# osqp/OSQP.jl

Hardware: AMD Instinct MI355X
Metric: ADMM iterations/sec (higher is better)
Workload: dtype f64; 1 GPU; rand-1e6; n=1000000, m=1000000, nnz_A=1000000000, nnz_P_full=1000749500, nnz_P_triu=500874750, backend=pcg, check_termination=25, adaptive_rho_interval=50, instances=1

## Files before the change

### osqp.jl_amd/csrc/abi.hip

```cpp
#include "engine.hpp"
#include "symbolic.hpp"

#include <cstring>
#include <thread>
#include <atomic>
#include <cmath>

using namespace oq;

namespace {

struct Impl {
  Engine eng;
  OSQPData data;
  OSQPSettings settings;
  OSQPSolution solution;
  OSQPInfo info;
};

Engine *E(OSQPWorkspace *w) { return &((Impl *)w->impl)->eng; }

struct DeviceGuard {
  int prev = -1;
  explicit DeviceGuard(int want) {
// ... 378 lines not shown
              const int k = R.rowid[r];
              same = k >= 0 && k < S.N && !seen[k];
              if (!same) break;
              seen[k] = 1;
              const int64_t len = S.Rp[k + 1] - S.Rp[k];
              same = c + (size_t)len <= R.cols[b].size();
              if (!same) break;
              std::vector<int> got(R.cols[b].begin() + c, R.cols[b].begin() + c + len);
              std::sort(got.begin(), got.end());
              same = std::equal(got.begin(), got.end(), S.Rj.begin() + S.Rp[k]);
              c += (size_t)len;
            }
          }
        }
        Supernodes T2;
        build_supernodes(S2, (int)smax, T2, false, true);
        same = same && T2.count == T.count && T2.ptr == T.ptr && T2.piv == T.piv && T2.up == T.up && T2.lvl_ptr == T.lvl_ptr && T2.woff == T.woff;
        for (int q = 0; q < S.N && same; q++) same = T2.Fp[q + 1] - T2.Fp[q] >= T.Fp[q + 1] - T.Fp[q] && T2.Gp[q + 1] - T2.Gp[q] >= T.Gp[q + 1] - T.Gp[q];
      }
      symbolic_complete(S2);
      same = same && !S2.lean && S2.Lp == S.Lp && S2.Li == S.Li && S2.Rp == S.Rp && S2.Rj == S.Rj && S2.Rmap == S.Rmap && S2.PtoL == S.PtoL &&
             S2.AtoL == S.AtoL;
      out[14] = same ? 1.0 : 0.0;
    }
    out[5] = (double)T.Fp[S.N]; out[6] = (double)T.wdoubles; out[7] = largest; out[8] = ok ? 1.0 : 0.0; out[9] = (double)inside;
    int lD, cD, kD;
    choose_dense_top(S, 512, getenv("OSQP_AMD_DENSE_MAX") ? atoi(getenv("OSQP_AMD_DENSE_MAX")) : 12288, 1024, 32, lD, cD, kD);
    out[10] = level_solve_cost_us(S, 512, lD, kD); out[11] = supernode_solve_cost_us(T, 256);
    out[12] = supernodes_pay(S, T, 512, lD, kD, 256) ? 1.0 : 0.0;
    if (getenv("OSQP_AMD_PROBE_VERBOSE"))
      for (int L = 0; L < T.nlev; L++) {
        int64_t rows = 0, pre = 0, post = 0, back = 0;
        int smax_l = 0;
        for (int J = T.lvl_ptr[L]; J < T.lvl_ptr[L + 1]; J++) {
          smax_l = std::max(smax_l, T.ptr[J + 1] - T.ptr[J]);
          for (int q = T.ptr[J]; q < T.ptr[J + 1]; q++) { rows++; pre += T.Fsplit[q] - T.Fp[q]; post += T.Fp[q + 1] - T.Fsplit[q]; back += T.Gp[q + 1] - T.Gp[q]; }
        }
        {
          int64_t cnt[3] = {0, 0, 0}, rw[3] = {0, 0, 0}, ef[3] = {0, 0, 0}, eb[3] = {0, 0, 0}, mxb[3] = {0, 0, 0};
          for (int J = T.lvl_ptr[L]; J < T.lvl_ptr[L + 1]; J++) {
            const int64_t sz = T.ptr[J + 1] - T.ptr[J];
            const int c = sz == 1 ? 0 : (sz <= Supernodes::kSmall ? 1 : 2);
            cnt[c]++; rw[c] += sz;
            for (int q = T.ptr[J]; q < T.ptr[J + 1]; q++) { ef[c] += T.Fp[q + 1] - T.Fp[q]; eb[c] += T.Gp[q + 1] - T.Gp[q]; mxb[c] = std::max<int64_t>(mxb[c], T.Gp[q + 1] - T.Gp[q]); }
          }
          for (int c = 0; c < 3; c++)
// ... 300 lines not shown
```

### osqp.jl_amd/csrc/direct.hip

```cpp
#include <climits>
#include <cstring>
#include <cmath>

#include "engine.hpp"
#include "symbolic.hpp"
#include "mfront.hpp"
#include "mfront_big.hpp"

namespace oq {

namespace {

constexpr int kChainRows = 512;
constexpr int kChainThreads = 1024;

}
}

#include "direct_factor_kernels.hpp"
#include "direct_dense_kernels.hpp"
#include "direct_level_kernels.hpp"
#include "direct_sn_kernels.hpp"
#include "direct_sndense_kernels.hpp"

// ... 19 lines not shown
  double *Sinv = nullptr;
  int ldD = 0;
  std::vector<char> long_rows;
  size_t w_half = 0;
  std::vector<Step> fwd, bwd;
  long long factorizations = 0;
  bool sn = false;
  Supernodes T;
  DevBuf<int> sn_ptr, sn_piv, perm_s, pinv_s, sn_Fj, sn_Gi, sn_up, sn_waits, sn_pending, sn_ready;
  int *sn_fault = nullptr, *sn_fault_host = nullptr;
  ~LdlFactor() { if (sn_fault_host) (void)hipHostFree(sn_fault_host); }
  bool faulted() const {
    if (!sn_fault_host) return false;
    if (inject_fault) { inject_fault = false; *sn_fault_host = 1; }
    return *(volatile int *)sn_fault_host != 0;
  }
  mutable bool inject_fault = getenv("OSQP_AMD_SNODE_FAULT_TEST") && atoi(getenv("OSQP_AMD_SNODE_FAULT_TEST")) == 1;
  bool sn_tree = false;
  int sn_tree_threads = 1024;
  int sn_tree_grid = 0;
  DevBuf<int> sn_ticket;
  int sn_tree_L0 = 1;
  DevBuf<int64_t> sn_woff, sn_wmap, sn_Fp, sn_Fpos, sn_Gp, sn_Gpos, sn_Fsplit;
  DevBuf<double> sn_Wc, sn_Wr, sn_Fx, sn_Gx, sn_Dinv;
  std::vector<int> sn_lanes_f, sn_lanes_b;
  bool mf = false;
  DevBuf<int> mf_snof, mf_slot, mf_bsz, mf_chp, mf_chl, mf_list, mf_err;
  DevBuf<int64_t> mf_uoff, mf_reloff;
  DevBuf<uint16_t> mf_rel, mf_loc;
  DevBuf<double> mf_U;
  struct MfLaunch { int cls, off, count, fcap; int tile_off = 0, tile_count = 0, chunk_off = 0, chunk_count = 0; };
  std::vector<MfLaunch> mf_launches;
  DevBuf<int64_t> mf_poff;
  DevBuf<double> mf_panel;
  DevBuf<int64_t> mf_ct0;
  DevBuf<int> mf_tiles, mf_chunks, mf_wide, mf_nwide;
  std::vector<int> mfh_chunks;
  std::vector<int64_t> mfh_poff;
  std::vector<char> mf_is_big;
  std::vector<int> mfh_tiles;
  int mf_big_count = 0, mf_big_fmax = 0;
  int mf_fmax = 0;
  bool mf_ok = false;
  int snd_L0 = -1, snd_J0 = -1, snd_q0 = 0, snd_K = 0;
  int snd_nb = 0, snd_nv = 0, snd_ntiles = 0;
  bool snd_vec_mode = false;
// ... 243 lines not shown
      HIP_CHECK(hipHostGetDevicePointer((void **)&sn_fault, sn_fault_host, 0));
    }
    up64(sn_woff, T.woff);
    if (lean) lean_device_lists(q_upper);
    else {
      if (!mf_ok) up64(sn_wmap, T.wmap);
      up64(sn_Fp, T.Fp); up64(sn_Fpos, T.Fpos); up64(sn_Gp, T.Gp); up64(sn_Gpos, T.Gpos); up64(sn_Fsplit, T.Fsplit);
    }
    sn_lanes_f.assign(T.nlev, 1); sn_lanes_b.assign(T.nlev, 1);
    for (int L = 0; L < T.nlev; L++) {
      int64_t ef = 0, eb = 0, rows = 0;
      for (int J = T.lvl_ptr[L]; J < T.lvl_ptr[L + 1]; J++) {
        const int q0 = T.ptr[J], q1 = T.ptr[J + 1];
        ef += T.Fp[q1] - T.Fp[q0]; eb += T.Gp[q1] - T.Gp[q0]; rows += q1 - q0;
      }
      sn_lanes_f[L] = pick((double)ef / (double)std::max<int64_t>(1, rows));
      sn_lanes_b[L] = pick((double)eb / (double)std::max<int64_t>(1, rows));
    }
    std::vector<int> ps(N), pis(N);
    for (int q = 0; q < N; q++) { ps[q] = S.perm[T.piv[q]]; pis[ps[q]] = q; }
    up32(perm_s, ps); up32(pinv_s, pis);
    sn_Wc.alloc(T.woff[T.count]); sn_Wr.alloc(T.woff[T.count]);
    sn_Fx.alloc(std::max<size_t>(1, (size_t)T.Fp[N])); sn_Gx.alloc(std::max<size_t>(1, (size_t)T.Gp[N])); sn_Dinv.alloc(N);
    e.sync();
    std::vector<int64_t>().swap(T.wmap); std::vector<int64_t>().swap(T.Fpos); std::vector<int64_t>().swap(T.Gpos);
    std::vector<int>().swap(T.Fj); std::vector<int>().swap(T.Gi);
  }

  int sn_top_Jt = -1, sn_top_level = -1;
  DevBuf<int64_t> sn_Ftop;
  DevBuf<int> sn_tchp, sn_tchl;
  DevBuf<double> sn_uvec;
  SnTop sn_top_args() const {
    if (sn_top_Jt < 0 || !mf) return SnTop{-1, nullptr, nullptr, nullptr, nullptr, nullptr, nullptr, nullptr, nullptr, nullptr};
    return SnTop{sn_top_Jt, sn_Ftop.get(), sn_tchp.get(), sn_tchl.get(), mf_bsz.get(), mf_reloff.get(), mf_rel.get(), mf_poff.get(), mf_panel.get(), sn_uvec.get()};
  }
  void setup_top() {
    sn_top_Jt = -1; sn_top_level = -1;
    if (!mf || !sn_tree || mf_big_count == 0) return;
    if (getenv("OSQP_AMD_SNODE_TOP") && atoi(getenv("OSQP_AMD_SNODE_TOP")) == 0) return;
    if (snd_K && !(getenv("OSQP_AMD_SNODE_TOP") && atoi(getenv("OSQP_AMD_SNODE_TOP")) == 1)) return;
    int Lt = T.nlev;
    for (int L = T.nlev - 1; L >= std::max(1, sn_tree_L0); L--) {
      bool all = true;
      for (int J = T.lvl_ptr[L]; J < T.lvl_ptr[L + 1] && all; J++) all = mfh_poff[J + 1] > mfh_poff[J] && mfh_bsz[J] <= 4096;
      if (!all) break;
// ... 774 lines not shown
      std::swap(cur, nxt);
    }
    Sinv = cur;
  }

#define OQ_CHAIN_CASE(UU, LL)                                                                                                      \
  if (t.U == UU && t.L == LL) {                                                                                                     \
    if (fwd_) OQ_LAUNCH((k_fwd_chain_lds<UU, LL>), dim3(1), dim3(kChainThreads), 0, s, t.a, t.b, level_ptr.get(), Rsplit.get(),    \
                        Rp.get(), Rj.get(), Rx.get(), bp.get());                                                                    \
    else OQ_LAUNCH((k_bwd_chain_lds<UU, LL>), dim3(1), dim3(kChainThreads), 0, s, t.a, t.b, level_ptr.get(), Lp.get(),            \
                   Lsplit.get(), Li.get(), Lx.get(), bp.get());                                                                     \
    return;                                                                                                                         \
  }
  void launch_chain(const Step &t, bool fwd_, hipStream_t s) {
    OQ_CHAIN_CASE(2, 64) OQ_CHAIN_CASE(4, 64) OQ_CHAIN_CASE(8, 64)
    OQ_CHAIN_CASE(2, 16) OQ_CHAIN_CASE(4, 16) OQ_CHAIN_CASE(8, 16)
    OQ_CHAIN_CASE(2, 4) OQ_CHAIN_CASE(4, 4)
    throw Error(6, "internal: no chain kernel for this step");
  }
#undef OQ_CHAIN_CASE
  void launch_fwd_chain(const Step &t, hipStream_t s) { launch_chain(t, true, s); }
  void launch_bwd_chain(const Step &t, hipStream_t s) { launch_chain(t, false, s); }

#define OQ_SN_LEVEL_W(LA, FWD, GS, JA, JB)                                                                                            \
  OQ_LAUNCH((k_sn_level_w<LA, FWD, GS>), dim3(((JB) - (JA) + 4 * (64 / GS) - 1) / (4 * (64 / GS))), dim3(kSnThreads), 0, s, JA, JB, sn_ptr.get(), \
            sn_woff.get(), FWD ? sn_Fp.get() : sn_Gp.get(), FWD ? sn_Fj.get() : sn_Gi.get(), FWD ? sn_Fx.get() : sn_Gx.get(),          \
            FWD ? sn_Wc.get() : sn_Wr.get(), sn_Dinv.get(), bp.get())
#define OQ_SN_LEVEL(LA, FWD, L)                                                                                                   \
  do {                                                                                                                            \
    const int cnt_ = T.lvl_ptr[L + 1] - T.lvl_ptr[L];                                                                             \
    if (cnt_ >= sn_wave_min_fixed) {                                                                                                \
      const int mid_ = T.lvl_ptr[L] + T.lvl_small[L];                                                                             \
                             \
      const int ones_ = sn_singles ? T.lvl_single[L] : 0, first_ = T.lvl_ptr[L] + ((FWD && L > 0) ? 0 : ones_);                   \
      if (!FWD && ones_ > 0)                                                                                                      \
        OQ_LAUNCH(k_sn_single_bwd, dim3(blocks_for(ones_)), dim3(kBlock), 0, s, T.ptr[T.lvl_ptr[L]], ones_, sn_Gp.get(),          \
                  sn_Gi.get(), sn_Gx.get(), sn_Dinv.get(), bp.get());                                                             \
               \
      if (mid_ > first_) OQ_SN_LEVEL_W((LA == 64 ? 16 : (LA == 16 ? 4 : LA)), FWD, 16, first_, mid_);                             \
      if (T.lvl_ptr[L + 1] > mid_ && !lvl_fold.empty() && lvl_fold[L])                                                            \
        OQ_LAUNCH((k_sn_level_wf<FWD, true>), dim3((T.lvl_ptr[L + 1] - mid_ + 3) / 4), dim3(kSnThreads), 0, s, mid_,               \
                  T.lvl_ptr[L + 1], sn_ptr.get(), sn_woff.get(), FWD ? sn_Fp.get() : sn_Gp.get(), FWD ? sn_Fj.get() : sn_Gi.get(),  \
                  FWD ? sn_Fx.get() : sn_Gx.get(), FWD ? sn_Wc.get() : sn_Wr.get(), sn_Dinv.get(), bp.get());                      \
      else if (T.lvl_ptr[L + 1] > mid_ && sn_flat && !(FWD && L == 0))                                                            \
        OQ_LAUNCH((k_sn_level_wf<FWD, false>), dim3((T.lvl_ptr[L + 1] - mid_ + 3) / 4), dim3(kSnThreads), 0, s, mid_,              \
                  T.lvl_ptr[L + 1], sn_ptr.get(), sn_woff.get(), FWD ? sn_Fp.get() : sn_Gp.get(), FWD ? sn_Fj.get() : sn_Gi.get(),  \
                  FWD ? sn_Fx.get() : sn_Gx.get(), FWD ? sn_Wc.get() : sn_Wr.get(), sn_Dinv.get(), bp.get());                      \
      else if (T.lvl_ptr[L + 1] > mid_) OQ_SN_LEVEL_W((LA == 64 ? 16 : (LA == 16 ? 4 : LA)), FWD, 64, mid_, T.lvl_ptr[L + 1]);     \
    } else if (sn_flat && !lvl_fold.empty() && lvl_fold[L])                                                                       \
      OQ_LAUNCH((k_sn_level_f<FWD, true>), dim3(cnt_), dim3(kSnThreads), 0, s, T.lvl_ptr[L], sn_ptr.get(), sn_woff.get(),          \
                FWD ? sn_Fp.get() : sn_Gp.get(), FWD ? sn_Fj.get() : sn_Gi.get(), FWD ? sn_Fx.get() : sn_Gx.get(),                  \
                FWD ? sn_Wc.get() : sn_Wr.get(), sn_Dinv.get(), bp.get());                                                        \
    else if (sn_flat)                                                                                                             \
      OQ_LAUNCH((k_sn_level_f<FWD, false>), dim3(cnt_), dim3(kSnThreads), 0, s, T.lvl_ptr[L], sn_ptr.get(), sn_woff.get(),         \
                FWD ? sn_Fp.get() : sn_Gp.get(), FWD ? sn_Fj.get() : sn_Gi.get(), FWD ? sn_Fx.get() : sn_Gx.get(),                  \
                FWD ? sn_Wc.get() : sn_Wr.get(), sn_Dinv.get(), bp.get());                                                        \
    else if (cnt_ >= kSnBusyLevel)           \
      OQ_LAUNCH((k_sn_level<(LA == 64 ? 16 : (LA == 16 ? 4 : LA)), FWD>), dim3(cnt_), dim3(kSnThreads), 0, s, T.lvl_ptr[L], sn_ptr.get(), \
                sn_woff.get(), FWD ? sn_Fp.get() : sn_Gp.get(), FWD ? sn_Fj.get() : sn_Gi.get(), FWD ? sn_Fx.get() : sn_Gx.get(),  \
                FWD ? sn_Wc.get() : sn_Wr.get(), sn_Dinv.get(), bp.get());                                                        \
    else                                                                                                                          \
      OQ_LAUNCH((k_sn_level<LA, FWD>), dim3(cnt_), dim3(kSnThreads), 0, s, T.lvl_ptr[L], sn_ptr.get(),                           \
                sn_woff.get(), FWD ? sn_Fp.get() : sn_Gp.get(), FWD ? sn_Fj.get() : sn_Gi.get(), FWD ? sn_Fx.get() : sn_Gx.get(),  \
                FWD ? sn_Wc.get() : sn_Wr.get(), sn_Dinv.get(), bp.get());                                                        \
  } while (0)
#define OQ_SN_TREE(FWD)                                                                                                           \
  if (sn_tree_threads == 512) OQ_SN_TREE_N(FWD, 512); else OQ_SN_TREE_N(FWD, 1024)
#define OQ_SN_TREE_N(FWD, NT_)                                                                                                    \
  OQ_LAUNCH((k_sn_tree<FWD, NT_>), dim3(sn_tree_grid ? sn_tree_grid : sn_j_end() - T.lvl_ptr[sn_tree_L0]), dim3(NT_), 0, s, sn_top_args(), T.lvl_ptr[sn_tree_L0], sn_j_end(), sn_ptr.get(),    \
            sn_woff.get(), FWD ? sn_Fp.get() : sn_Gp.get(), FWD ? sn_Fsplit.get() : sn_Gp.get(), FWD ? sn_Fj.get() : sn_Gi.get(),      \
            FWD ? sn_Fx.get() : sn_Gx.get(), FWD ? sn_Wc.get() : sn_Wr.get(), sn_Dinv.get(), sn_up.get(), sn_waits.get(),          \
            FWD ? sn_pending.get() : sn_ready.get(), sn_fault, bp.get(), sn_tree_grid ? sn_ticket.get() + (FWD ? 0 : 1) : (int *)nullptr)
  const bool sn_fold = !(getenv("OSQP_AMD_SNODE_FOLD") && atoi(getenv("OSQP_AMD_SNODE_FOLD")) == 0) &&
                       !(getenv("OSQP_AMD_SNODE_FLAT") && atoi(getenv("OSQP_AMD_SNODE_FLAT")) == 0);
  const int sn_wave_min_fixed = sn_wave_min();
  const bool sn_fold_wg = !(getenv("OSQP_AMD_SNODE_FOLD") && atoi(getenv("OSQP_AMD_SNODE_FOLD")) == 2);
  std::vector<char> lvl_fold;
  void fold_blocks(hipStream_t s) {
    if (!sn || !sn_fold) return;
    if (lvl_fold.empty()) {
      lvl_fold.assign(T.nlev, 0);
      for (int L = 0; L < T.nlev; L++) {
        const int cnt = T.lvl_ptr[L + 1] - T.lvl_ptr[L], mid = T.lvl_ptr[L] + T.lvl_small[L];
        lvl_fold[L] = (cnt >= sn_wave_min_fixed ? T.lvl_ptr[L + 1] > mid : sn_fold_wg) && !(sn_tree && L >= sn_tree_L0);
      }
    }
    for (int L = 0; L < sn_l_end(); L++) {
      const int cnt = T.lvl_ptr[L + 1] - T.lvl_ptr[L];
      const int mid = cnt >= sn_wave_min_fixed ? T.lvl_ptr[L] + T.lvl_small[L] : T.lvl_ptr[L];
      if (!lvl_fold[L]) continue;
      OQ_LAUNCH(k_sn_fold<true>, dim3(T.lvl_ptr[L + 1] - mid), dim3(64), 0, s, mid, sn_ptr.get(), sn_woff.get(), sn_Wc.get());
      OQ_LAUNCH(k_sn_fold<false>, dim3(T.lvl_ptr[L + 1] - mid), dim3(64), 0, s, mid, sn_ptr.get(), sn_woff.get(), sn_Wr.get());
    }
  }
  const bool sn_flat = !(getenv("OSQP_AMD_SNODE_FLAT") && atoi(getenv("OSQP_AMD_SNODE_FLAT")) == 0);
  const bool sn_singles = !(getenv("OSQP_AMD_SNODE_SINGLE") && atoi(getenv("OSQP_AMD_SNODE_SINGLE")) == 0);
  static int sn_wave_min() { const char *v = getenv("OSQP_AMD_SNODE_WAVE_MIN"); return v ? atoi(v) : kSnWaveLevel; }
  int sn_l_end() const { return snd_K ? snd_L0 : T.nlev; }
  int sn_j_end() const { return snd_K ? snd_J0 : T.count; }
  void run_supernodes() {
    hipStream_t s = e.stream;
    const bool tree = sn_tree && sn_tree_L0 < sn_l_end();
    const int plain = tree ? sn_tree_L0 : sn_l_end();
    for (int L = 0; L < plain; L++) switch (sn_lanes_f[L]) {
      case 1: OQ_SN_LEVEL(1, true, L); break;
      case 4: OQ_SN_LEVEL(4, true, L); break;
      case 16: OQ_SN_LEVEL(16, true, L); break;
      default: OQ_SN_LEVEL(64, true, L); break;
    }
    if (tree && sn_tree_grid) HIP_CHECK(hipMemsetAsync(sn_ticket.get(), 0, 2 * sizeof(int), s));
    if (tree) { OQ_SN_TREE(true); }
    if (snd_K) solve_dense_top(s, tree);
    if (tree) { OQ_SN_TREE(false); }
    for (int L = plain - 1; L >= 0; L--) switch (sn_lanes_b[L]) {
      case 1: OQ_SN_LEVEL(1, false, L); break;
      case 4: OQ_SN_LEVEL(4, false, L); break;
      case 16: OQ_SN_LEVEL(16, false, L); break;
      default: OQ_SN_LEVEL(64, false, L); break;
    }
  }
#undef OQ_SN_LEVEL
#undef OQ_SN_LEVEL_W
#undef OQ_SN_TREE
#undef OQ_SN_TREE_N

  void run_steps(bool skip_first_fwd = false, bool skip_last_bwd = false) {
    hipStream_t s = e.stream;
    if (sn) { run_supernodes(); return; }
    for (size_t si = 0; si < fwd.size(); si++) {
      const Step &t = fwd[si];
      if (si == 0 && skip_first_fwd) continue;
      if (t.kind == 1) {
        const int c0 = S.level_ptr[t.a], c1 = S.level_ptr[t.b];
        if (t.G == kBlock) OQ_LAUNCH(k_fwd_far<kBlock>, dim3(c1 - c0), dim3(kBlock), 0, s, c0, c1, Rp.get(), Rsplit.get(), Rj.get(), Rx.get(), bp.get(), (double *)nullptr);
        else OQ_LAUNCH(k_fwd_far<64>, dim3(blocks_for((int64_t)(c1 - c0) * 64)), dim3(kBlock), 0, s, c0, c1, Rp.get(), Rsplit.get(), Rj.get(), Rx.get(), bp.get(), (double *)nullptr);
        launch_fwd_chain(t, s);
        continue;
      }
      dim3 grid(blocks_for((int64_t)(t.b - t.a) * t.G)), block(kBlock);
      switch (t.G) {
      case 1: OQ_LAUNCH(k_fwd_level<1>, grid, block, 0, s, t.a, t.b, Rp.get(), Rj.get(), Rx.get(), bp.get()); break;
      case 4: OQ_LAUNCH(k_fwd_level<4>, grid, block, 0, s, t.a, t.b, Rp.get(), Rj.get(), Rx.get(), bp.get()); break;
      case 16: OQ_LAUNCH(k_fwd_level<16>, grid, block, 0, s, t.a, t.b, Rp.get(), Rj.get(), Rx.get(), bp.get()); break;
      default: OQ_LAUNCH(k_fwd_level<64>, grid, block, 0, s, t.a, t.b, Rp.get(), Rj.get(), Rx.get(), bp.get()); break;
      }
// ... 296 lines not shown
```

### osqp.jl_amd/csrc/direct_sn_kernels.hpp

```cpp
#pragma once
#include "engine.hpp"

namespace oq {
namespace {

constexpr int kSnMax = 64, kSnThreads = 256;
constexpr int kSnBusyLevel = 2048;
constexpr int kSnWaveLevel = 16384;

__global__ __launch_bounds__(kSnThreads) void k_sn_invert(const int *__restrict__ ptr, const int64_t *__restrict__ woff,
                                                          const int64_t *__restrict__ wmap, const double *__restrict__ Lx,
                                                          double *__restrict__ Wc, double *__restrict__ Wr) {
  __shared__ double Ld[kSnMax * kSnMax], Wd[kSnMax * kSnMax];
  const int J = blockIdx.x, s = ptr[J + 1] - ptr[J];
  const int64_t w0 = woff[J];
  for (int e = threadIdx.x; e < s * s; e += kSnThreads) {
    const int i = e / s, k = e - i * s;
    double v = 0.0;
    if (k < i) { const int64_t t = wmap[w0 + (int64_t)i * (i + 1) / 2 + k]; if (t >= 0) v = Lx[t]; }
    Ld[e] = v;
  }
  __syncthreads();
  if ((int)threadIdx.x < s) {
    const int j = threadIdx.x;
// ... 46 lines not shown
                                                         const double *__restrict__ Ex, const double *__restrict__ W,
                                                         const double *__restrict__ Dinv_s, double *__restrict__ b) {
  __shared__ double t[kSnMax];
  __shared__ double part[kSnThreads / 64][kSnMax];
  const int J = J0 + blockIdx.x, q0 = ptr[J], s = ptr[J + 1] - q0;
  {
    const int lane = threadIdx.x % LA;
    for (int a = threadIdx.x / LA; a < s; a += kSnThreads / LA) {
      const int q = q0 + a;
      double acc = gather_dot(Ep[q] + lane, Ep[q + 1], LA, Ej, Ex, b);
#pragma unroll
      for (int o = LA / 2; o > 0; o >>= 1) acc += __shfl_xor(acc, o);
      if (lane == 0) t[a] = (kForward ? b[q] : b[q] * Dinv_s[q]) - acc;
    }
  }
  __syncthreads();
  const double *Wj = W + woff[J];
  const int wv = threadIdx.x >> 6, a = threadIdx.x & 63;
  part[wv][a] = sn_block_row<kForward>(Wj, t, s, a, wv, kSnThreads / 64);
  __syncthreads();
  if (wv == 0 && a < s) b[q0 + a] = (part[0][a] + part[1][a]) + (part[2][a] + part[3][a]);
}

template <int LA, bool kForward, int GS>
__global__ __launch_bounds__(kSnThreads) void k_sn_level_w(int J0, int J1, const int *__restrict__ ptr, const int64_t *__restrict__ woff,
                                                           const int64_t *__restrict__ Ep, const int *__restrict__ Ej,
                                                           const double *__restrict__ Ex, const double *__restrict__ W,
                                                           const double *__restrict__ Dinv_s, double *__restrict__ b) {
  static_assert(LA <= GS, "the lanes of a row lie inside its supernode's group");
  constexpr int NG = 64 / GS, TS = GS == 64 ? kSnMax : GS;
  __shared__ double tt[kSnThreads / 64][NG][TS];
  const int wv = threadIdx.x >> 6, l64 = threadIdx.x & 63, g = l64 / GS, gl = l64 % GS;
  const int J = J0 + (blockIdx.x * (kSnThreads / 64) + wv) * NG + g;
  const bool live = J < J1;
  double *t = tt[wv][g];
  const int q0 = live ? ptr[J] : 0, s = live ? ptr[J + 1] - q0 : 0;
  {
    const int lane = gl % LA;
    for (int a = gl / LA; a < s; a += GS / LA) {
      const int q = q0 + a;
      double acc = gather_dot(Ep[q] + lane, Ep[q + 1], LA, Ej, Ex, b);
#pragma unroll
      for (int o = LA / 2; o > 0; o >>= 1) acc += __shfl_xor(acc, o);
      if (lane == 0) t[a] = (kForward ? b[q] : b[q] * Dinv_s[q]) - acc;
    }
  }
  __builtin_amdgcn_fence(__ATOMIC_RELEASE, "wavefront");
  __builtin_amdgcn_s_waitcnt(0xc07f);
  __builtin_amdgcn_wave_barrier();
  const double *Wj = W + (live ? woff[J] : 0);
  const double acc = sn_block_row<kForward>(Wj, t, s, gl, 0, 1);
  if (gl < s) b[q0 + gl] = acc;
}

constexpr int kSnFlatU = 8;
template <bool kForward, int DK>
__device__ __forceinline__ void sn_block_fold(const double *__restrict__ Wj, const double *t, int s, int gl, int k0, double &lo, double &hi);
template <bool kForward, bool kFold>
__global__ __launch_bounds__(kSnThreads) void k_sn_level_f(int J0, const int *__restrict__ ptr, const int64_t *__restrict__ woff,
                                                           const int64_t *__restrict__ Ep, const int *__restrict__ Ej,
                                                           const double *__restrict__ Ex, const double *__restrict__ W,
                                                           const double *__restrict__ Dinv_s, double *__restrict__ b) {
  constexpr int C = kSnThreads * kSnFlatU;
  __shared__ double prod[C];
  __shared__ double t[kSnMax];
  __shared__ double part[kSnThreads / 64][kSnMax];
  const int J = J0 + blockIdx.x, q0 = ptr[J], s = ptr[J + 1] - q0;
  const int tid = threadIdx.x, ra = tid >> 2, rk = tid & 3;
  const int64_t E0 = Ep[q0], E1 = Ep[q0 + s];
  int64_t r1 = 0, pos = 0;
  double rhs = 0.0;
  if (ra < s) {
    pos = Ep[q0 + ra] + rk; r1 = Ep[q0 + ra + 1];
// ... 28 lines not shown
  }
  __syncthreads();
  const double *Wj = W + woff[J];
  const int wv = tid >> 6, a = tid & 63;
  if (kFold) {
    double lo, hi;
    sn_block_fold<kForward, 8>(Wj, t, s, a, 2 * wv + (a >> 5), lo, hi);
    if (a < 32) { part[wv][a] = lo; part[wv][32 + a] = hi; }
    __syncthreads();
    const int h = (s + 1) >> 1;
    if (wv == 0 && a < h) {
      const double slo = (part[0][a] + part[1][a]) + (part[2][a] + part[3][a]);
      const double shi = (part[0][32 + a] + part[1][32 + a]) + (part[2][32 + a] + part[3][32 + a]);
      b[q0 + (kForward ? a : s - 1 - a)] = slo;
      if (a != s - 1 - a) b[q0 + (kForward ? s - 1 - a : a)] = shi;
    }
    return;
  }
  part[wv][a] = sn_block_row<kForward>(Wj, t, s, a, wv, kSnThreads / 64);
  __syncthreads();
  if (wv == 0 && a < s) b[q0 + a] = (part[0][a] + part[1][a]) + (part[2][a] + part[3][a]);
}
template <bool kForward, int DK>
__device__ __forceinline__ void sn_block_fold(const double *__restrict__ Wj, const double *t, int s, int gl, int k0, double &lo, double &hi) {
  const int h = (s + 1) >> 1, a = gl & 31, par = gl >> 5;
  lo = 0.0; hi = 0.0;
  if (a < h) {
    auto idx = [&](int k) { return kForward ? (k <= a ? k : k - a - 1) : (k <= a ? s - 1 - a + k : k - 1); };
    int k = k0;
    for (; k + 3 * DK <= s; k += 4 * DK) {
      const double w0 = Wj[k * h + a], w1 = Wj[(k + DK) * h + a], w2 = Wj[(k + 2 * DK) * h + a], w3 = Wj[(k + 3 * DK) * h + a];
      const double p0 = w0 * t[idx(k)], p1 = w1 * t[idx(k + DK)], p2 = w2 * t[idx(k + 2 * DK)], p3 = w3 * t[idx(k + 3 * DK)];
      if (k <= a) lo += p0; else hi += p0;
      if (k + DK <= a) lo += p1; else hi += p1;
      if (k + 2 * DK <= a) lo += p2; else hi += p2;
      if (k + 3 * DK <= a) lo += p3; else hi += p3;
    }
    for (; k <= s; k += DK) {
      const double p0 = Wj[k * h + a] * t[idx(k)];
      if (k <= a) lo += p0; else hi += p0;
    }
  }
  const double lo2 = __shfl_xor(lo, 32), hi2 = __shfl_xor(hi, 32);
  lo = par ? lo2 + lo : lo + lo2;
  hi = par ? hi2 + hi : hi + hi2;
}
template <bool kForward, bool kFold>
__global__ __launch_bounds__(kSnThreads) void k_sn_level_wf(int J0, int J1, const int *__restrict__ ptr, const int64_t *__restrict__ woff,
                                                            const int64_t *__restrict__ Ep, const int *__restrict__ Ej,
                                                            const double *__restrict__ Ex, const double *__restrict__ W,
                                                            const double *__restrict__ Dinv_s, double *__restrict__ b) {
  constexpr int C = 64 * kSnFlatU;
  __shared__ double prod_all[kSnThreads / 64][C];
  __shared__ double tt[kSnThreads / 64][kSnMax];
  const int wv = threadIdx.x >> 6, gl = threadIdx.x & 63;
  const int J = J0 + blockIdx.x * (kSnThreads / 64) + wv;
  if (J >= J1) return;
  double *prod = prod_all[wv], *t = tt[wv];
  const int q0 = ptr[J], s = ptr[J + 1] - q0;
  const int64_t E0 = Ep[q0], E1 = Ep[q0 + s];
  int64_t r1 = 0, pos = 0;
  double rhs = 0.0;
  if (gl < s) {
    pos = Ep[q0 + gl]; r1 = Ep[q0 + gl + 1];
    rhs = kForward ? b[q0 + gl] : b[q0 + gl] * Dinv_s[q0 + gl];
  }
  double acc = 0.0;
  for (int64_t base = E0; base < E1; base += C) {
// ... 6 lines not shown
      idx[u] = ok ? Ej[e] : -1;
      val[u] = ok ? Ex[e] : 0.0;
    }
#pragma unroll
    for (int u = 0; u < kSnFlatU; u++) bv[u] = idx[u] >= 0 ? b[idx[u]] : 0.0;
#pragma unroll
    for (int u = 0; u < kSnFlatU; u++) prod[u * 64 + gl] = val[u] * bv[u];
    __builtin_amdgcn_fence(__ATOMIC_RELEASE, "wavefront");
    __builtin_amdgcn_s_waitcnt(0xc07f);
    __builtin_amdgcn_wave_barrier();
    const int64_t end = r1 < base + C ? r1 : base + C;
    for (; pos < end; pos++) acc += prod[pos - base];
    __builtin_amdgcn_fence(__ATOMIC_RELEASE, "wavefront");
    __builtin_amdgcn_wave_barrier();
  }
  if (gl < s) t[gl] = rhs - acc;
  __builtin_amdgcn_fence(__ATOMIC_RELEASE, "wavefront");
  __builtin_amdgcn_s_waitcnt(0xc07f);
  __builtin_amdgcn_wave_barrier();
  const double *Wj = W + woff[J];
  if (kFold) {
    double lo, hi;
    sn_block_fold<kForward, 2>(Wj, t, s, gl, gl >> 5, lo, hi);
    const int a = gl & 31, h = (s + 1) >> 1;
    if (gl < h) {
      b[q0 + (kForward ? a : s - 1 - a)] = lo;
      if (a != s - 1 - a) b[q0 + (kForward ? s - 1 - a : a)] = hi;
    }
    return;
  }
  const double out = sn_block_row<kForward>(Wj, t, s, gl, 0, 1);
  if (gl < s) b[q0 + gl] = out;
}
template <bool kForward>
__global__ __launch_bounds__(64) void k_sn_fold(int J0, const int *__restrict__ ptr, const int64_t *__restrict__ woff, double *__restrict__ W) {
  __shared__ double tri[kSnMax * (kSnMax + 1) / 2];
  const int J = J0 + blockIdx.x, s = ptr[J + 1] - ptr[J], gl = threadIdx.x;
  double *Wj = W + woff[J];
  const int nel = s * (s + 1) / 2, h = (s + 1) >> 1;
  for (int e = gl; e < nel; e += 64) tri[e] = Wj[e];
  __builtin_amdgcn_fence(__ATOMIC_RELEASE, "wavefront");
  __builtin_amdgcn_s_waitcnt(0xc07f);
  __builtin_amdgcn_wave_barrier();
  auto at = [&](int r, int c) { return kForward ? tri[c * s - c * (c - 1) / 2 + (r - c)] : tri[r * (r + 1) / 2 + c]; };
  for (int e = gl; e < (s + 1) * h; e += 64) {
    const int k = e / h, a = e - k * h;
// ... 192 lines not shown
```

Before: 85.83 iterations/s.

## Add software-pipelined supernode level solve kernels with packed per-supernode records

```diff
diff --git a/osqp.jl_amd/csrc/abi.hip b/osqp.jl_amd/csrc/abi.hip
--- a/osqp.jl_amd/csrc/abi.hip
+++ b/osqp.jl_amd/csrc/abi.hip
@@ -424,6 +424,22 @@
       same = same && !S2.lean && S2.Lp == S.Lp && S2.Li == S.Li && S2.Rp == S.Rp && S2.Rj == S.Rj && S2.Rmap == S.Rmap && S2.PtoL == S.PtoL &&
              S2.AtoL == S.AtoL;
       out[14] = same ? 1.0 : 0.0;
+    }
+    if (count >= 17) {
+      std::vector<int> mark((size_t)S.N, -1);
+      double cells[2] = {0.0, 0.0};
+      for (int dir = 0; dir < 2; dir++) {
+        std::fill(mark.begin(), mark.end(), -1);
+        const std::vector<int64_t> &Ep = dir == 0 ? T.Gp : T.Fp;
+        const std::vector<int> &Ej = dir == 0 ? T.Gi : T.Fj;
+        for (int J = 0; J < T.count; J++) {
+          int64_t distinct = 0;
+          for (int64_t i = Ep[T.ptr[J]]; i < Ep[T.ptr[J + 1]]; i++)
+            if (mark[Ej[i]] != J) { mark[Ej[i]] = J; distinct++; }
+          cells[dir] += (double)(T.ptr[J + 1] - T.ptr[J]) * (double)distinct;
+        }
+      }
+      out[15] = cells[0]; out[16] = cells[1];
     }
     out[5] = (double)T.Fp[S.N]; out[6] = (double)T.wdoubles; out[7] = largest; out[8] = ok ? 1.0 : 0.0; out[9] = (double)inside;
     int lD, cD, kD;
diff --git a/osqp.jl_amd/csrc/direct.hip b/osqp.jl_amd/csrc/direct.hip
--- a/osqp.jl_amd/csrc/direct.hip
+++ b/osqp.jl_amd/csrc/direct.hip
@@ -65,6 +65,7 @@
   DevBuf<int> sn_ticket;
   int sn_tree_L0 = 1;
   DevBuf<int64_t> sn_woff, sn_wmap, sn_Fp, sn_Fpos, sn_Gp, sn_Gpos, sn_Fsplit;
+  DevBuf<SnRec> sn_rec_f, sn_rec_b;
   DevBuf<double> sn_Wc, sn_Wr, sn_Fx, sn_Gx, sn_Dinv;
   std::vector<int> sn_lanes_f, sn_lanes_b;
   bool mf = false;
@@ -354,6 +355,12 @@
     up32(perm_s, ps); up32(pinv_s, pis);
     sn_Wc.alloc(T.woff[T.count]); sn_Wr.alloc(T.woff[T.count]);
     sn_Fx.alloc(std::max<size_t>(1, (size_t)T.Fp[N])); sn_Gx.alloc(std::max<size_t>(1, (size_t)T.Gp[N])); sn_Dinv.alloc(N);
+    if (sn_pipe & 1) {
+      sn_rec_f.alloc(T.count); sn_rec_b.alloc(T.count);
+      OQ_LAUNCH(k_sn_records, dim3(blocks_for(T.count)), dim3(kBlock), 0, s, T.count, (const int *)sn_ptr.get(), (const int64_t *)sn_Fp.get(),
+                (const int64_t *)sn_Gp.get(), (const int64_t *)sn_woff.get(), sn_rec_f.get(), sn_rec_b.get());
+    }
+    if (getenv("OSQP_AMD_SETUP_TRACE")) fprintf(stderr, "[supernodes] level kernels: pipe=%d\n", sn_pipe);
     e.sync();
     std::vector<int64_t>().swap(T.wmap); std::vector<int64_t>().swap(T.Fpos); std::vector<int64_t>().swap(T.Gpos);
     std::vector<int>().swap(T.Fj); std::vector<int>().swap(T.Gi);
@@ -1174,10 +1181,37 @@
   void launch_fwd_chain(const Step &t, hipStream_t s) { launch_chain(t, true, s); }
   void launch_bwd_chain(const Step &t, hipStream_t s) { launch_chain(t, false, s); }
 
-#define OQ_SN_LEVEL_W(LA, FWD, GS, JA, JB)                                                                                            \
-  OQ_LAUNCH((k_sn_level_w<LA, FWD, GS>), dim3(((JB) - (JA) + 4 * (64 / GS) - 1) / (4 * (64 / GS))), dim3(kSnThreads), 0, s, JA, JB, sn_ptr.get(), \
-            sn_woff.get(), FWD ? sn_Fp.get() : sn_Gp.get(), FWD ? sn_Fj.get() : sn_Gi.get(), FWD ? sn_Fx.get() : sn_Gx.get(),          \
-            FWD ? sn_Wc.get() : sn_Wr.get(), sn_Dinv.get(), bp.get())
+#define OQ_SN_ARGS(FWD)                                                                                                           \
+  sn_ptr.get(), sn_woff.get(), FWD ? sn_Fp.get() : sn_Gp.get(), FWD ? sn_Fj.get() : sn_Gi.get(), FWD ? sn_Fx.get() : sn_Gx.get(),   \
+      FWD ? sn_Wc.get() : sn_Wr.get(), sn_Dinv.get(), bp.get()
+#define OQ_SN_REC(FWD) (const SnRec *)(FWD ? sn_rec_f.get() : sn_rec_b.get())
+#define OQ_SN_LEVEL_W_(LA, FWD, GS, JA, JB, REC)                                                                                    \
+  OQ_LAUNCH((k_sn_level_w<LA, FWD, GS, REC>), dim3(((JB) - (JA) + 4 * (64 / GS) - 1) / (4 * (64 / GS))), dim3(kSnThreads), 0, s, JA, JB, \
+            OQ_SN_REC(FWD), OQ_SN_ARGS(FWD))
+#define OQ_SN_LEVEL_W(LA, FWD, GS, JA, JB)                                                                                          \
+  do {                                                                                                                              \
+    if (sn_pipe & 1) OQ_SN_LEVEL_W_(LA, FWD, GS, JA, JB, true); else OQ_SN_LEVEL_W_(LA, FWD, GS, JA, JB, false);                    \
+  } while (0)
+#define OQ_SN_PIPED(KERN, FWD, FOLD, ...)                                                                                           \
+  switch (sn_pipe) {                                                                                                                \
+  case 1: OQ_LAUNCH((KERN<FWD, FOLD, 1>), __VA_ARGS__, OQ_SN_REC(FWD), OQ_SN_ARGS(FWD)); break;                                     \
+  case 2: OQ_LAUNCH((KERN<FWD, FOLD, 2>), __VA_ARGS__, OQ_SN_REC(FWD), OQ_SN_ARGS(FWD)); break;                                     \
+  case 3: OQ_LAUNCH((KERN<FWD, FOLD, 3>), __VA_ARGS__, OQ_SN_REC(FWD), OQ_SN_ARGS(FWD)); break;                                     \
+  case 4: OQ_LAUNCH((KERN<FWD, FOLD, 4>), __VA_ARGS__, OQ_SN_REC(FWD), OQ_SN_ARGS(FWD)); break;                                     \
+  case 5: OQ_LAUNCH((KERN<FWD, FOLD, 5>), __VA_ARGS__, OQ_SN_REC(FWD), OQ_SN_ARGS(FWD)); break;                                     \
+  case 6: OQ_LAUNCH((KERN<FWD, FOLD, 6>), __VA_ARGS__, OQ_SN_REC(FWD), OQ_SN_ARGS(FWD)); break;                                     \
+  default: OQ_LAUNCH((KERN<FWD, FOLD, 7>), __VA_ARGS__, OQ_SN_REC(FWD), OQ_SN_ARGS(FWD)); break;                                    \
+  }
+#define OQ_SN_LEVEL_WF(FWD, FOLD, JA, JB)                                                                                           \
+  do {                                                                                                                              \
+    if (sn_pipe) { OQ_SN_PIPED(k_sn_level_wfp, FWD, FOLD, dim3(((JB) - (JA) + 3) / 4), dim3(kSnThreads), 0, s, JA, JB) }            \
+    else OQ_LAUNCH((k_sn_level_wf<FWD, FOLD>), dim3(((JB) - (JA) + 3) / 4), dim3(kSnThreads), 0, s, JA, JB, OQ_SN_ARGS(FWD));       \
+  } while (0)
+#define OQ_SN_LEVEL_F(FWD, FOLD, L)                                                                                                 \
+  do {                                                                                                                              \
+    if (sn_pipe) { OQ_SN_PIPED(k_sn_level_fp, FWD, FOLD, dim3(cnt_), dim3(kSnThreads), 0, s, T.lvl_ptr[L]) }                        \
+    else OQ_LAUNCH((k_sn_level_f<FWD, FOLD>), dim3(cnt_), dim3(kSnThreads), 0, s, T.lvl_ptr[L], OQ_SN_ARGS(FWD));                   \
+  } while (0)
 #define OQ_SN_LEVEL(LA, FWD, L)                                                                                                   \
   do {                                                                                                                            \
     const int cnt_ = T.lvl_ptr[L + 1] - T.lvl_ptr[L];                                                                             \
@@ -1190,31 +1224,14 @@
                   sn_Gi.get(), sn_Gx.get(), sn_Dinv.get(), bp.get());                                                             \
                \
       if (mid_ > first_) OQ_SN_LEVEL_W((LA == 64 ? 16 : (LA == 16 ? 4 : LA)), FWD, 16, first_, mid_);                             \
-      if (T.lvl_ptr[L + 1] > mid_ && !lvl_fold.empty() && lvl_fold[L])                                                            \
-        OQ_LAUNCH((k_sn_level_wf<FWD, true>), dim3((T.lvl_ptr[L + 1] - mid_ + 3) / 4), dim3(kSnThreads), 0, s, mid_,               \
-                  T.lvl_ptr[L + 1], sn_ptr.get(), sn_woff.get(), FWD ? sn_Fp.get() : sn_Gp.get(), FWD ? sn_Fj.get() : sn_Gi.get(),  \
-                  FWD ? sn_Fx.get() : sn_Gx.get(), FWD ? sn_Wc.get() : sn_Wr.get(), sn_Dinv.get(), bp.get());                      \
-      else if (T.lvl_ptr[L + 1] > mid_ && sn_flat && !(FWD && L == 0))                                                            \
-        OQ_LAUNCH((k_sn_level_wf<FWD, false>), dim3((T.lvl_ptr[L + 1] - mid_ + 3) / 4), dim3(kSnThreads), 0, s, mid_,              \
-                  T.lvl_ptr[L + 1], sn_ptr.get(), sn_woff.get(), FWD ? sn_Fp.get() : sn_Gp.get(), FWD ? sn_Fj.get() : sn_Gi.get(),  \
-                  FWD ? sn_Fx.get() : sn_Gx.get(), FWD ? sn_Wc.get() : sn_Wr.get(), sn_Dinv.get(), bp.get());                      \
+      if (T.lvl_ptr[L + 1] > mid_ && !lvl_fold.empty() && lvl_fold[L]) OQ_SN_LEVEL_WF(FWD, true, mid_, T.lvl_ptr[L + 1]);         \
+      else if (T.lvl_ptr[L + 1] > mid_ && sn_flat && !(FWD && L == 0)) OQ_SN_LEVEL_WF(FWD, false, mid_, T.lvl_ptr[L + 1]);        \
       else if (T.lvl_ptr[L + 1] > mid_) OQ_SN_LEVEL_W((LA == 64 ? 16 : (LA == 16 ? 4 : LA)), FWD, 64, mid_, T.lvl_ptr[L + 1]);     \
-    } else if (sn_flat && !lvl_fold.empty() && lvl_fold[L])                                                                       \
-      OQ_LAUNCH((k_sn_level_f<FWD, true>), dim3(cnt_), dim3(kSnThreads), 0, s, T.lvl_ptr[L], sn_ptr.get(), sn_woff.get(),          \
-                FWD ? sn_Fp.get() : sn_Gp.get(), FWD ? sn_Fj.get() : sn_Gi.get(), FWD ? sn_Fx.get() : sn_Gx.get(),                  \
-                FWD ? sn_Wc.get() : sn_Wr.get(), sn_Dinv.get(), bp.get());                                                        \
-    else if (sn_flat)                                                                                                             \
-      OQ_LAUNCH((k_sn_level_f<FWD, false>), dim3(cnt_), dim3(kSnThreads), 0, s, T.lvl_ptr[L], sn_ptr.get(), sn_woff.get(),         \
-                FWD ? sn_Fp.get() : sn_Gp.get(), FWD ? sn_Fj.get() : sn_Gi.get(), FWD ? sn_Fx.get() : sn_Gx.get(),                  \
-                FWD ? sn_Wc.get() : sn_Wr.get(), sn_Dinv.get(), bp.get());                                                        \
+    } else if (sn_flat && !lvl_fold.empty() && lvl_fold[L]) OQ_SN_LEVEL_F(FWD, true, L);                                          \
+    else if (sn_flat) OQ_SN_LEVEL_F(FWD, false, L);                                                                               \
     else if (cnt_ >= kSnBusyLevel)           \
-      OQ_LAUNCH((k_sn_level<(LA == 64 ? 16 : (LA == 16 ? 4 : LA)), FWD>), dim3(cnt_), dim3(kSnThreads), 0, s, T.lvl_ptr[L], sn_ptr.get(), \
-                sn_woff.get(), FWD ? sn_Fp.get() : sn_Gp.get(), FWD ? sn_Fj.get() : sn_Gi.get(), FWD ? sn_Fx.get() : sn_Gx.get(),  \
-                FWD ? sn_Wc.get() : sn_Wr.get(), sn_Dinv.get(), bp.get());                                                        \
-    else                                                                                                                          \
-      OQ_LAUNCH((k_sn_level<LA, FWD>), dim3(cnt_), dim3(kSnThreads), 0, s, T.lvl_ptr[L], sn_ptr.get(),                           \
-                sn_woff.get(), FWD ? sn_Fp.get() : sn_Gp.get(), FWD ? sn_Fj.get() : sn_Gi.get(), FWD ? sn_Fx.get() : sn_Gx.get(),  \
-                FWD ? sn_Wc.get() : sn_Wr.get(), sn_Dinv.get(), bp.get());                                                        \
+      OQ_LAUNCH((k_sn_level<(LA == 64 ? 16 : (LA == 16 ? 4 : LA)), FWD>), dim3(cnt_), dim3(kSnThreads), 0, s, T.lvl_ptr[L], OQ_SN_ARGS(FWD)); \
+    else OQ_LAUNCH((k_sn_level<LA, FWD>), dim3(cnt_), dim3(kSnThreads), 0, s, T.lvl_ptr[L], OQ_SN_ARGS(FWD));                     \
   } while (0)
 #define OQ_SN_TREE(FWD)                                                                                                           \
   if (sn_tree_threads == 512) OQ_SN_TREE_N(FWD, 512); else OQ_SN_TREE_N(FWD, 1024)
@@ -1245,6 +1262,7 @@
       OQ_LAUNCH(k_sn_fold<false>, dim3(T.lvl_ptr[L + 1] - mid), dim3(64), 0, s, mid, sn_ptr.get(), sn_woff.get(), sn_Wr.get());
     }
   }
+  const int sn_pipe = getenv("OSQP_AMD_SNODE_PIPE") ? (atoi(getenv("OSQP_AMD_SNODE_PIPE")) & 7) : 7;
   const bool sn_flat = !(getenv("OSQP_AMD_SNODE_FLAT") && atoi(getenv("OSQP_AMD_SNODE_FLAT")) == 0);
   const bool sn_singles = !(getenv("OSQP_AMD_SNODE_SINGLE") && atoi(getenv("OSQP_AMD_SNODE_SINGLE")) == 0);
   static int sn_wave_min() { const char *v = getenv("OSQP_AMD_SNODE_WAVE_MIN"); return v ? atoi(v) : kSnWaveLevel; }
@@ -1272,7 +1290,13 @@
     }
   }
 #undef OQ_SN_LEVEL
+#undef OQ_SN_LEVEL_F
+#undef OQ_SN_LEVEL_WF
+#undef OQ_SN_PIPED
 #undef OQ_SN_LEVEL_W
+#undef OQ_SN_LEVEL_W_
+#undef OQ_SN_REC
+#undef OQ_SN_ARGS
 #undef OQ_SN_TREE
 #undef OQ_SN_TREE_N
 
diff --git a/osqp.jl_amd/csrc/direct_sn_kernels.hpp b/osqp.jl_amd/csrc/direct_sn_kernels.hpp
--- a/osqp.jl_amd/csrc/direct_sn_kernels.hpp
+++ b/osqp.jl_amd/csrc/direct_sn_kernels.hpp
@@ -92,8 +92,10 @@
   if (wv == 0 && a < s) b[q0 + a] = (part[0][a] + part[1][a]) + (part[2][a] + part[3][a]);
 }
 
-template <int LA, bool kForward, int GS>
-__global__ __launch_bounds__(kSnThreads) void k_sn_level_w(int J0, int J1, const int *__restrict__ ptr, const int64_t *__restrict__ woff,
+struct SnRec { int q0, s; int64_t e0, e1, woff; };
+static_assert(sizeof(SnRec) == 32, "one aligned 32-byte load per supernode");
+template <int LA, bool kForward, int GS, bool kRec>
+__global__ __launch_bounds__(kSnThreads) void k_sn_level_w(int J0, int J1, const SnRec *__restrict__ rec, const int *__restrict__ ptr, const int64_t *__restrict__ woff,
                                                            const int64_t *__restrict__ Ep, const int *__restrict__ Ej,
                                                            const double *__restrict__ Ex, const double *__restrict__ W,
                                                            const double *__restrict__ Dinv_s, double *__restrict__ b) {
@@ -104,7 +106,10 @@
   const int J = J0 + (blockIdx.x * (kSnThreads / 64) + wv) * NG + g;
   const bool live = J < J1;
   double *t = tt[wv][g];
-  const int q0 = live ? ptr[J] : 0, s = live ? ptr[J + 1] - q0 : 0;
+  int q0 = 0, s = 0;
+  int64_t w0 = 0;
+  if (kRec) { if (live) { q0 = rec[J].q0; s = rec[J].s; w0 = rec[J].woff; } }
+  else { q0 = live ? ptr[J] : 0; s = live ? ptr[J + 1] - q0 : 0; }
   {
     const int lane = gl % LA;
     for (int a = gl / LA; a < s; a += GS / LA) {
@@ -118,7 +123,7 @@
   __builtin_amdgcn_fence(__ATOMIC_RELEASE, "wavefront");
   __builtin_amdgcn_s_waitcnt(0xc07f);
   __builtin_amdgcn_wave_barrier();
-  const double *Wj = W + (live ? woff[J] : 0);
+  const double *Wj = W + (kRec ? w0 : (live ? woff[J] : 0));
   const double acc = sn_block_row<kForward>(Wj, t, s, gl, 0, 1);
   if (gl < s) b[q0 + gl] = acc;
 }
@@ -193,28 +198,58 @@
   if (wv == 0 && a < s) b[q0 + a] = (part[0][a] + part[1][a]) + (part[2][a] + part[3][a]);
 }
 template <bool kForward, int DK>
-__device__ __forceinline__ void sn_block_fold(const double *__restrict__ Wj, const double *t, int s, int gl, int k0, double &lo, double &hi) {
-  const int h = (s + 1) >> 1, a = gl & 31, par = gl >> 5;
-  lo = 0.0; hi = 0.0;
-  if (a < h) {
-    auto idx = [&](int k) { return kForward ? (k <= a ? k : k - a - 1) : (k <= a ? s - 1 - a + k : k - 1); };
-    int k = k0;
-    for (; k + 3 * DK <= s; k += 4 * DK) {
-      const double w0 = Wj[k * h + a], w1 = Wj[(k + DK) * h + a], w2 = Wj[(k + 2 * DK) * h + a], w3 = Wj[(k + 3 * DK) * h + a];
-      const double p0 = w0 * t[idx(k)], p1 = w1 * t[idx(k + DK)], p2 = w2 * t[idx(k + 2 * DK)], p3 = w3 * t[idx(k + 3 * DK)];
-      if (k <= a) lo += p0; else hi += p0;
-      if (k + DK <= a) lo += p1; else hi += p1;
-      if (k + 2 * DK <= a) lo += p2; else hi += p2;
-      if (k + 3 * DK <= a) lo += p3; else hi += p3;
-    }
-    for (; k <= s; k += DK) {
-      const double p0 = Wj[k * h + a] * t[idx(k)];
-      if (k <= a) lo += p0; else hi += p0;
-    }
-  }
+__device__ __forceinline__ void sn_fold_steps(const double *__restrict__ Wj, const double *t, int s, int h, int a, int k, double &lo, double &hi) {
+  auto idx = [&](int k) { return kForward ? (k <= a ? k : k - a - 1) : (k <= a ? s - 1 - a + k : k - 1); };
+  for (; k + 3 * DK <= s; k += 4 * DK) {
+    const double w0 = Wj[k * h + a], w1 = Wj[(k + DK) * h + a], w2 = Wj[(k + 2 * DK) * h + a], w3 = Wj[(k + 3 * DK) * h + a];
+    const double p0 = w0 * t[idx(k)], p1 = w1 * t[idx(k + DK)], p2 = w2 * t[idx(k + 2 * DK)], p3 = w3 * t[idx(k + 3 * DK)];
+    if (k <= a) lo += p0; else hi += p0;
+    if (k + DK <= a) lo += p1; else hi += p1;
+    if (k + 2 * DK <= a) lo += p2; else hi += p2;
+    if (k + 3 * DK <= a) lo += p3; else hi += p3;
+  }
+  for (; k <= s; k += DK) {
+    const double p0 = Wj[k * h + a] * t[idx(k)];
+    if (k <= a) lo += p0; else hi += p0;
+  }
+}
+__device__ __forceinline__ void sn_fold_meet(int par, double &lo, double &hi) {
   const double lo2 = __shfl_xor(lo, 32), hi2 = __shfl_xor(hi, 32);
   lo = par ? lo2 + lo : lo + lo2;
   hi = par ? hi2 + hi : hi + hi2;
+}
+template <bool kForward, int DK>
+__device__ __forceinline__ void sn_block_fold(const double *__restrict__ Wj, const double *t, int s, int gl, int k0, double &lo, double &hi) {
+  const int h = (s + 1) >> 1, a = gl & 31;
+  lo = 0.0; hi = 0.0;
+  if (a < h) sn_fold_steps<kForward, DK>(Wj, t, s, h, a, k0, lo, hi);
+  sn_fold_meet(gl >> 5, lo, hi);
+}
+template <int DK, int NP>
+__device__ __forceinline__ void sn_fold_prefetch(const double *__restrict__ Wj, int s, int gl, int k0, double (&w)[NP]) {
+  const int h = (s + 1) >> 1, a = gl & 31;
+#pragma unroll
+  for (int i = 0; i < NP; i++) {
+    const int k = k0 + i * DK;
+    w[i] = (a < h && k <= s) ? Wj[k * h + a] : 0.0;
+  }
+}
+template <bool kForward, int DK, int NP>
+__device__ __forceinline__ void sn_block_fold_pre(const double *__restrict__ Wj, const double *t, int s, int gl, int k0, const double (&w)[NP], double &lo, double &hi) {
+  const int h = (s + 1) >> 1, a = gl & 31;
+  lo = 0.0; hi = 0.0;
+  if (a < h) {
+#pragma unroll
+    for (int i = 0; i < NP; i++) {
+      const int k = k0 + i * DK;
+      if (k <= s) {
+        const double p = w[i] * t[kForward ? (k <= a ? k : k - a - 1) : (k <= a ? s - 1 - a + k : k - 1)];
+        if (k <= a) lo += p; else hi += p;
+      }
+    }
+    sn_fold_steps<kForward, DK>(Wj, t, s, h, a, k0 + NP * DK, lo, hi);
+  }
+  sn_fold_meet(gl >> 5, lo, hi);
 }
 template <bool kForward, bool kFold>
 __global__ __launch_bounds__(kSnThreads) void k_sn_level_wf(int J0, int J1, const int *__restrict__ ptr, const int64_t *__restrict__ woff,
@@ -267,6 +302,213 @@
   if (kFold) {
     double lo, hi;
     sn_block_fold<kForward, 2>(Wj, t, s, gl, gl >> 5, lo, hi);
+    const int a = gl & 31, h = (s + 1) >> 1;
+    if (gl < h) {
+      b[q0 + (kForward ? a : s - 1 - a)] = lo;
+      if (a != s - 1 - a) b[q0 + (kForward ? s - 1 - a : a)] = hi;
+    }
+    return;
+  }
+  const double out = sn_block_row<kForward>(Wj, t, s, gl, 0, 1);
+  if (gl < s) b[q0 + gl] = out;
+}
+__global__ __launch_bounds__(kBlock) void k_sn_records(int count, const int *__restrict__ ptr, const int64_t *__restrict__ Fp,
+                                                       const int64_t *__restrict__ Gp, const int64_t *__restrict__ woff,
+                                                       SnRec *__restrict__ rf, SnRec *__restrict__ rb) {
+  const int J = blockIdx.x * kBlock + threadIdx.x;
+  if (J >= count) return;
+  const int q0 = ptr[J], s = ptr[J + 1] - q0;
+  rf[J] = SnRec{q0, s, Fp[q0], Fp[q0 + s], woff[J]};
+  rb[J] = SnRec{q0, s, Gp[q0], Gp[q0 + s], woff[J]};
+}
+template <bool kRec>
+__device__ __forceinline__ SnRec sn_head(int J, const SnRec *__restrict__ rec, const int *__restrict__ ptr, const int64_t *__restrict__ woff,
+                                         const int64_t *__restrict__ Ep) {
+  if (kRec) return rec[J];
+  const int q0 = ptr[J], s = ptr[J + 1] - q0;
+  return SnRec{q0, s, Ep[q0], Ep[q0 + s], woff[J]};
+}
+__device__ __forceinline__ int sn_clamped(int piece, int lane, int last, int bytes) {
+  return piece * bytes < 4096 ? piece + min(lane, last - piece) : min(piece + lane, last);
+}
+constexpr int kSnPreF = 9, kSnPreW = 8;
+template <bool kForward, bool kFold, int kPipe>
+__global__ __launch_bounds__(kSnThreads, 8) void k_sn_level_fp(int J0, const SnRec *__restrict__ rec, const int *__restrict__ ptr,
+                                                               const int64_t *__restrict__ woff, const int64_t *__restrict__ Ep,
+                                                               const int *__restrict__ Ej, const double *__restrict__ Ex,
+                                                               const double *__restrict__ W, const double *__restrict__ Dinv_s,
+                                                               double *__restrict__ b) {
+  constexpr bool kPre = (kPipe & 2) && kFold, kAhead = (kPipe & 4) != 0;
+  constexpr int C = kSnThreads * kSnFlatU;
+  __shared__ double prod[C];
+  __shared__ double t[kSnMax];
+  __shared__ double part[kSnThreads / 64][kSnMax];
+  const int J = J0 + blockIdx.x;
+  const SnRec r = sn_head<(kPipe & 1) != 0>(J, rec, ptr, woff, Ep);
+  const int q0 = r.q0, s = r.s;
+  const int64_t E0 = r.e0, E1 = r.e1;
+  const int tid = threadIdx.x, ra = tid >> 2, rk = tid & 3, wv = tid >> 6, a = tid & 63;
+  const double *Wj = W + r.woff;
+  const int rem0 = (int)(E1 - E0 < C ? E1 - E0 : C);
+  int idx[kSnFlatU];
+  double wpre[kSnPreF];
+  if (kAhead) {
+#pragma unroll
+    for (int u = 0; u < kSnFlatU; u++) idx[u] = u * kSnThreads + tid < rem0 ? Ej[E0 + u * kSnThreads + tid] : q0;
+  }
+  const int qr = q0 + (ra < s ? ra : s - 1);
+  int64_t pos = Ep[qr];
+  const int64_t r1 = Ep[qr + 1];
+  double rhs = 0.0;
+  double acc = 0.0;
+  auto chunk = [&](const int64_t base, const bool last) __attribute__((always_inline)) {
+    const int rem = (int)(E1 - base < 2 * C ? E1 - base : 2 * C);
+    const int *Ejb = Ej + base;
+    const double *Exb = Ex + base;
+    double val[kSnFlatU], bv[kSnFlatU];
+    int nidx[kSnFlatU];
+    if (!kAhead) {
+#pragma unroll
+      for (int u = 0; u < kSnFlatU; u++) idx[u] = (!last || u * kSnThreads + tid < rem) ? Ejb[u * kSnThreads + tid] : q0;
+    }
+#pragma unroll
+    for (int u = 0; u < kSnFlatU; u++) bv[u] = (!last || u * kSnThreads + tid < rem) ? b[idx[u]] : 0.0;
+    __builtin_amdgcn_sched_barrier(0);
+    if (last) rhs = kForward ? b[qr] : b[qr] * Dinv_s[qr];
+#pragma unroll
+    for (int u = 0; u < kSnFlatU; u++) val[u] = (!last || u * kSnThreads + tid < rem) ? Exb[u * kSnThreads + tid] : 0.0;
+    __builtin_amdgcn_sched_barrier(0);
+    if (kAhead && !last) {
+#pragma unroll
+      for (int u = 0; u < kSnFlatU; u++) nidx[u] = Ejb[sn_clamped(C + u * kSnThreads, tid, rem - 1, 4)];
+    }
+#pragma unroll
+    for (int u = 0; u < kSnFlatU; u++) prod[u * kSnThreads + tid] = val[u] * bv[u];
+    if (kPre && last) sn_fold_prefetch<8, kSnPreF>(Wj, s, a, 2 * wv + (a >> 5), wpre);
+    __syncthreads();
+    const int64_t end = ra < s ? (r1 < base + C ? r1 : base + C) : 0;
+    for (; pos + rk < end; pos += 4) acc += prod[pos + rk - base];
+    __syncthreads();
+    if (kAhead && !last) {
+#pragma unroll
+      for (int u = 0; u < kSnFlatU; u++) idx[u] = nidx[u];
+    }
+  };
+  int64_t base = E0;
+  for (; base + C < E1; base += C) chunk(base, false);
+  if (base < E1) chunk(base, true);
+  else {
+    rhs = kForward ? b[qr] : b[qr] * Dinv_s[qr];
+    if (kPre) sn_fold_prefetch<8, kSnPreF>(Wj, s, a, 2 * wv + (a >> 5), wpre);
+  }
+  {
+    const double a1 = __shfl_xor(acc, 1);
+    const double pair = (rk & 1) ? a1 + acc : acc + a1;
+    const double other = __shfl_xor(pair, 2);
+    const double sum = (rk & 2) ? other + pair : pair + other;
+    if (rk == 0 && ra < s) t[ra] = rhs - sum;
+  }
+  __syncthreads();
+  if (kFold) {
+    double lo, hi;
+    if (kPre) sn_block_fold_pre<kForward, 8, kSnPreF>(Wj, t, s, a, 2 * wv + (a >> 5), wpre, lo, hi);
+    else sn_block_fold<kForward, 8>(Wj, t, s, a, 2 * wv + (a >> 5), lo, hi);
+    if (a < 32) { part[wv][a] = lo; part[wv][32 + a] = hi; }
+    __syncthreads();
+    const int h = (s + 1) >> 1;
+    if (wv == 0 && a < h) {
+      const double slo = (part[0][a] + part[1][a]) + (part[2][a] + part[3][a]);
+      const double shi = (part[0][32 + a] + part[1][32 + a]) + (part[2][32 + a] + part[3][32 + a]);
+      b[q0 + (kForward ? a : s - 1 - a)] = slo;
+      if (a != s - 1 - a) b[q0 + (kForward ? s - 1 - a : a)] = shi;
+    }
+    return;
+  }
+  part[wv][a] = sn_block_row<kForward>(Wj, t, s, a, wv, kSnThreads / 64);
+  __syncthreads();
+  if (wv == 0 && a < s) b[q0 + a] = (part[0][a] + part[1][a]) + (part[2][a] + part[3][a]);
+}
+template <bool kForward, bool kFold, int kPipe>
+__global__ __launch_bounds__(kSnThreads, 8) void k_sn_level_wfp(int J0, int J1, const SnRec *__restrict__ rec, const int *__restrict__ ptr,
+                                                                const int64_t *__restrict__ woff, const int64_t *__restrict__ Ep,
+                                                                const int *__restrict__ Ej, const double *__restrict__ Ex,
+                                                                const double *__restrict__ W, const double *__restrict__ Dinv_s,
+                                                                double *__restrict__ b) {
+  constexpr bool kPre = (kPipe & 2) && kFold, kAhead = (kPipe & 4) != 0;
+  constexpr int C = 64 * kSnFlatU;
+  __shared__ double prod_all[kSnThreads / 64][C];
+  __shared__ double tt[kSnThreads / 64][kSnMax];
+  const int wv = __builtin_amdgcn_readfirstlane(threadIdx.x >> 6), gl = threadIdx.x & 63;
+  const int J = J0 + blockIdx.x * (kSnThreads / 64) + wv;
+  if (J >= J1) return;
+  double *prod = prod_all[wv], *t = tt[wv];
+  const SnRec r = sn_head<(kPipe & 1) != 0>(J, rec, ptr, woff, Ep);
+  const int q0 = r.q0, s = r.s;
+  const int64_t E0 = r.e0, E1 = r.e1;
+  const double *Wj = W + r.woff;
+  const int rem0 = (int)(E1 - E0 < C ? E1 - E0 : C);
+  int idx[kSnFlatU];
+  double wpre[kSnPreW];
+  if (kAhead) {
+#pragma unroll
+    for (int u = 0; u < kSnFlatU; u++) idx[u] = u * 64 + gl < rem0 ? Ej[E0 + u * 64 + gl] : q0;
+  }
+  const int qr = q0 + (gl < s ? gl : s - 1);
+  int64_t pos = Ep[qr];
+  const int64_t r1 = Ep[qr + 1];
+  double rhs = 0.0;
+  double acc = 0.0;
+  auto chunk = [&](const int64_t base, const bool last) __attribute__((always_inline)) {
+    const int rem = (int)(E1 - base < 2 * C ? E1 - base : 2 * C);
+    const int *Ejb = Ej + base;
+    const double *Exb = Ex + base;
+    double val[kSnFlatU], bv[kSnFlatU];
+    int nidx[kSnFlatU];
+    if (!kAhead) {
+#pragma unroll
+      for (int u = 0; u < kSnFlatU; u++) idx[u] = (!last || u * 64 + gl < rem) ? Ejb[u * 64 + gl] : q0;
+    }
+#pragma unroll
+    for (int u = 0; u < kSnFlatU; u++) bv[u] = (!last || u * 64 + gl < rem) ? b[idx[u]] : 0.0;
+    __builtin_amdgcn_sched_barrier(0);
+    if (last) rhs = kForward ? b[qr] : b[qr] * Dinv_s[qr];
+#pragma unroll
+    for (int u = 0; u < kSnFlatU; u++) val[u] = (!last || u * 64 + gl < rem) ? Exb[u * 64 + gl] : 0.0;
+    __builtin_amdgcn_sched_barrier(0);
+    if (kAhead && !last) {
+#pragma unroll
+      for (int u = 0; u < kSnFlatU; u++) nidx[u] = Ejb[sn_clamped(C + u * 64, gl, rem - 1, 4)];
+    }
+#pragma unroll
+    for (int u = 0; u < kSnFlatU; u++) prod[u * 64 + gl] = val[u] * bv[u];
+    if (kPre && last) sn_fold_prefetch<2, kSnPreW>(Wj, s, gl, gl >> 5, wpre);
+    __builtin_amdgcn_fence(__ATOMIC_RELEASE, "wavefront");
+    __builtin_amdgcn_s_waitcnt(0xc07f);
+    __builtin_amdgcn_wave_barrier();
+    const int64_t end = gl < s ? (r1 < base + C ? r1 : base + C) : 0;
+    for (; pos < end; pos++) acc += prod[pos - base];
+    __builtin_amdgcn_fence(__ATOMIC_RELEASE, "wavefront");
+    __builtin_amdgcn_wave_barrier();
+    if (kAhead && !last) {
+#pragma unroll
+      for (int u = 0; u < kSnFlatU; u++) idx[u] = nidx[u];
+    }
+  };
+  int64_t base = E0;
+  for (; base + C < E1; base += C) chunk(base, false);
+  if (base < E1) chunk(base, true);
+  else {
+    rhs = kForward ? b[qr] : b[qr] * Dinv_s[qr];
+    if (kPre) sn_fold_prefetch<2, kSnPreW>(Wj, s, gl, gl >> 5, wpre);
+  }
+  if (gl < s) t[gl] = rhs - acc;
+  __builtin_amdgcn_fence(__ATOMIC_RELEASE, "wavefront");
+  __builtin_amdgcn_s_waitcnt(0xc07f);
+  __builtin_amdgcn_wave_barrier();
+  if (kFold) {
+    double lo, hi;
+    if (kPre) sn_block_fold_pre<kForward, 2, kSnPreW>(Wj, t, s, gl, gl >> 5, wpre, lo, hi);
+    else sn_block_fold<kForward, 2>(Wj, t, s, gl, gl >> 5, lo, hi);
     const int a = gl & 31, h = (s + 1) >> 1;
     if (gl < h) {
       b[q0 + (kForward ? a : s - 1 - a)] = lo;
```

Measured after the change: 85.85 iterations/s, median of 2. About the same (+0.0%).
